# jason-gideon/GPUMounter

Hardware: AMD Instinct MI355X
Metric: p50_gpu_attach_latency_ms (lower is better)
Workload: dtype none

## Files before the change

### gpumounter_amd/_native.py

```python
from __future__ import annotations

import ctypes as C
import os
import subprocess
import threading
from typing import Optional

LIB_DIR = os.path.join(os.path.dirname(os.path.abspath(__file__)), "_lib")
NATIVE_DIR = os.path.join(os.path.dirname(os.path.dirname(os.path.abspath(__file__))), "native")

_lock = threading.Lock()
_libs: dict = {}


class NativeError(RuntimeError):
    pass


def lib_path(name: str) -> str:
    return os.path.join(LIB_DIR, name)


def build(target: str = "all", quiet: bool = True) -> None:
    import fcntl
# ... 79 lines not shown
    _fields_ = [("type", C.c_char), ("access", C.c_uint8), ("allow", C.c_uint8),
                ("pad", C.c_uint8), ("major", C.c_int32), ("minor", C.c_int32)]


class DevNode(C.Structure):
    _fields_ = [("path", C.c_char * 112), ("major", C.c_uint32), ("minor", C.c_uint32),
                ("mode", C.c_uint32), ("uid", C.c_int32), ("gid", C.c_int32)]


class BpfTiming(C.Structure):
    _fields_ = [("query_ns", C.c_uint64), ("map_ns", C.c_uint64), ("build_ns", C.c_uint64),
                ("load_ns", C.c_uint64), ("attach_ns", C.c_uint64), ("programs", C.c_uint32),
                ("insns", C.c_uint32)]


HOST_ABI_VERSION = 6
GM_ACC_MKNOD, GM_ACC_READ, GM_ACC_WRITE = 1, 2, 4
GM_DEV_EMULATE, GM_DEV_VIA_SETNS, GM_DEV_REPLACE, GM_DEV_BIND = 1, 2, 4, 8


def host() -> C.CDLL:
    lib = _load("libgm_host.so", "host")
    if not getattr(lib, "_gm_typed", False):
        abi = lib.gm_host_abi_version()
        if abi != HOST_ABI_VERSION:
            raise RuntimeError(f"libgm_host.so ABI {abi} != {HOST_ABI_VERSION} expected: stale "
                               f"build, run `make -C native`")
        lib.gm_cg1_apply.argtypes = [C.c_char_p, C.POINTER(DevRule), C.c_int]
        lib.gm_cg1_format_rule.argtypes = [C.POINTER(DevRule), C.c_char_p, C.c_int]
        lib.gm_bpf_dev_build.argtypes = [C.POINTER(DevRule), C.c_int, C.c_int, C.c_int,
                                         C.POINTER(C.c_uint64), C.c_int]
# ... 21 lines not shown
        lib.gm_bpf_dev_set_at.argtypes = [C.c_char_p, C.c_uint32, C.POINTER(C.c_uint32),
                                          C.c_uint32, C.POINTER(C.c_uint32),
                                          C.POINTER(C.c_uint32)]
        lib.gm_bpf_dev_last_timing.argtypes = [C.POINTER(BpfTiming)]
        lib.gm_bpf_dev_last_timing.restype = None
        lib.gm_devnodes_create.argtypes = [C.c_int, C.c_char_p, C.POINTER(DevNode), C.c_int,
                                           C.c_int, C.POINTER(C.c_int)]
        lib.gm_devnodes_remove.argtypes = lib.gm_devnodes_create.argtypes
        lib.gm_devnodes_guard.argtypes = [C.c_char_p]
        lib.gm_devnodes_stage.argtypes = [C.c_char_p, C.c_int]
        lib.gm_devnode_stat.argtypes = [C.c_int, C.c_char_p, C.c_char_p, C.c_int,
                                        C.POINTER(C.c_int), C.POINTER(C.c_uint32),
                                        C.POINTER(C.c_uint32), C.POINTER(C.c_uint32)]
        lib.gm_devnodes_present.argtypes = [C.c_int, C.c_char_p, C.POINTER(DevNode), C.c_int,
                                            C.c_int, C.POINTER(C.c_uint8)]
        lib.gm_proc_dev_users.argtypes = [C.c_uint32, C.c_uint32, C.POINTER(C.c_int32), C.c_int,
                                          C.POINTER(C.c_int)]
        lib.gm_proc_scan_devs.argtypes = [C.POINTER(C.c_int32), C.c_int, C.POINTER(C.c_uint32),
                                          C.c_int, C.POINTER(C.c_uint8), C.POINTER(C.c_int32)]
        lib.gm_proc_filter_dev_users.argtypes = [C.POINTER(C.c_int32), C.c_int, C.c_uint32,
                                                 C.c_uint32, C.POINTER(C.c_int32)]
        lib.gm_proc_read_pids.argtypes = [C.c_char_p, C.POINTER(C.c_int32), C.c_int,
                                          C.POINTER(C.c_int)]
        lib.gm_sd_get_device_allow.argtypes = [C.c_char_p, C.c_char_p, C.c_char_p, C.c_int,
                                               C.c_char_p, C.c_int]
        lib.gm_sd_set_device_allow.argtypes = [C.c_char_p, C.c_char_p, C.POINTER(C.c_char_p),
                                               C.POINTER(C.c_char_p), C.c_int, C.c_int,
                                               C.c_char_p, C.c_int]
        lib.gm_sd_unit_path.argtypes = [C.c_char_p, C.c_char_p, C.c_int]
        lib.gm_roctx_push.argtypes = [C.c_char_p]
# ... 217 lines not shown
```

### gpumounter_amd/node/cgroup.py

```python
from __future__ import annotations

import ctypes as C
import errno
import functools
import glob
import json
import os
from abc import ABC, abstractmethod
from typing import Dict, FrozenSet, Iterable, List, Optional, Sequence, Set, Tuple

from gpumounter_amd import _native
from gpumounter_amd.models.device import DeviceNode
from gpumounter_amd.models.pod import (QOS_BESTEFFORT, QOS_BURSTABLE, ContainerRef, qos_class,
                                       uid_of)
from gpumounter_amd.node import bpfvm
from gpumounter_amd.utils import log, trace

_log = log.get("node.cgroup")

RUNTIME_SCOPE_PREFIXES = ("cri-containerd-", "docker-", "crio-", "containerd-", "")
FAKE_MARKER = ".gm_fake"
BPF_STATE = "gm.bpf.json"


# ... 93 lines not shown
                ctrls = parts[1].split(",") if parts[1] else [""]
                if want_ctrl not in ctrls:
                    continue
                cand = os.path.join(self.base, parts[2].lstrip("/"))
                if os.path.isdir(cand):
                    return cand
        return None

    def forget(self, pod_uid: str) -> None:
        for k in [k for k in self._cache if k[0] == pod_uid]:
            del self._cache[k]

    @staticmethod
    def pids(cgdir: str, recursive: bool = True) -> List[int]:
        lib = _native.host()
        out: List[int] = []
        buf = (C.c_int32 * 4096)()
        n = C.c_int(0)
        stack = [cgdir]
        while stack:
            d = stack.pop()
            path = os.path.join(d, "cgroup.procs")
            rc = lib.gm_proc_read_pids(path.encode(), buf, 4096, C.byref(n))
            if rc < 0 and rc != -errno.ENOENT:
                raise CgroupError(f"read {path}: {os.strerror(-rc)}")
            if rc >= 0:
                out.extend(buf[:min(n.value, 4096)])
            if recursive:
                try:
                    with os.scandir(d) as it:
                        stack.extend(e.path for e in it if e.is_dir(follow_symlinks=False))
                except (FileNotFoundError, NotADirectoryError):
                    pass
        return sorted(set(out))


def rules_for(nodes: Iterable[DeviceNode], allow: bool, access: str = "rw") -> List[_native.DevRule]:
    acc = 0
    if "r" in access:
        acc |= _native.GM_ACC_READ
    if "w" in access:
        acc |= _native.GM_ACC_WRITE
    if "m" in access:
        acc |= _native.GM_ACC_MKNOD
    return [_native.DevRule(b"c", acc, 1 if allow else 0, 0, n.major, n.minor) for n in nodes]


def _rule_array(rules: Sequence[_native.DevRule]):
    arr = (_native.DevRule * max(len(rules), 1))()
# ... 442 lines not shown
```

### gpumounter_amd/node/devnodes.py

```python
from __future__ import annotations

import ctypes as C
import errno
import os
from dataclasses import dataclass
from typing import List, Optional, Sequence, Tuple

from gpumounter_amd import _native
from gpumounter_amd.models.device import DeviceNode
from gpumounter_amd.utils import log


class DevNodeError(RuntimeError):
    def __init__(self, msg: str, results: Sequence[int] = ()):
        super().__init__(msg)
        self.results = list(results)


@dataclass(frozen=True)
class Target:

    pid: int = 0
    root: str = ""


CREATED, PRESENT, SHARED_HOST = 0, 1, 2

_log = log.get("node.devnodes")


class DevNodeWriter:

    def __init__(self, mode: str = "procroot", host_dev: str = "", userns: str = "auto",
                 stage_dir: str = "", proc_root: str = "/proc") -> None:
        self.mode = mode
        self.userns = userns
        self.stage_dir = stage_dir
        self.proc_root = proc_root
        self._staged = False
        self._own_userns = self._userns_id("self")
        self.flags = 0
        if mode == "setns":
            self.flags |= _native.GM_DEV_VIA_SETNS
# ... 7 lines not shown

    @staticmethod
    def _array(nodes: Sequence[DeviceNode], owner: Tuple[int, int] = (-1, -1)):
        arr = (_native.DevNode * max(len(nodes), 1))()
        for i, n in enumerate(nodes):
            rel = n.path.lstrip("/").encode()
            if len(rel) >= 112:
                raise DevNodeError(f"path too long: {n.path}")
            arr[i].path = rel
            arr[i].major = n.major
            arr[i].minor = n.minor
            arr[i].mode = n.mode
            arr[i].uid, arr[i].gid = owner
        return arr

    def _mntns(self, pid) -> Optional[str]:
        try:
            return os.readlink(f"{self.proc_root}/{pid}/ns/mnt")
        except OSError:
            return None

    def root_pid(self, pids: Sequence[int]) -> int:
        if self.mode == "emulate":
            return pids[0] if pids else 0
        own = self._mntns("self")
        for pid in pids:
            ns = self._mntns(pid)
            if ns is not None and ns != own:
                return pid
        return 0

    def _userns_id(self, pid) -> Optional[Tuple[int, int]]:
        try:
            st = os.stat(f"{self.proc_root}/{pid}/ns/user")
        except OSError:
            return None
        return st.st_dev, st.st_ino

    def _bind(self, t: Target) -> bool:
        if self.userns == "bind":
            return True
        if self.userns != "auto" or self.mode == "emulate" or t.root or t.pid <= 0:
            return False
        theirs = self._userns_id(t.pid)
        return theirs is not None and self._own_userns is not None and theirs != self._own_userns
# ... 32 lines not shown
        self._staged = True

    def _call(self, t: Target):
        if not self._bind(t):
            return self.flags, (-1, -1)
        self._ensure_stage()
        return self.flags | _native.GM_DEV_BIND, self._mapped_root(t)

    def _target_args(self, t: Target) -> Tuple[int, Optional[bytes]]:
        if t.root:
            return 0, t.root.encode()
        if t.pid <= 0:
            raise DevNodeError("container has no process to resolve its root from "
                               "(empty cgroup.procs)")
        return t.pid, None

    def create(self, t: Target, nodes: Sequence[DeviceNode]) -> List[int]:
        if not nodes:
            return []
        pid, root = self._target_args(t)
        flags, owner = self._call(t)
        res = (C.c_int * len(nodes))()
        fails = _native.host().gm_devnodes_create(pid, root, self._array(nodes, owner),
                                                  len(nodes), flags, res)
        results = [int(res[i]) for i in range(len(nodes))]
        if fails:
            bad = [(n.path, os.strerror(-r)) for n, r in zip(nodes, results) if r < 0]
            what = "bind mount" if flags & _native.GM_DEV_BIND else "mknod"
            raise DevNodeError(f"{what} failed: {bad}", results)
        return results
# ... 44 lines not shown
        return kind in (1, 2) and ma == node.major and mi == node.minor

    def present_many(self, t: Target, nodes: Sequence[DeviceNode]) -> List[bool]:
        return [bool(s) for s in self.present_states(t, nodes)]

    def present_states(self, t: Target, nodes: Sequence[DeviceNode]) -> List[int]:
        if not nodes:
            return []
        pid, root = self._target_args(t)
        out = (C.c_uint8 * len(nodes))()
        rc = _native.host().gm_devnodes_present(pid, root, self._array(nodes), len(nodes),
                                                self._call(t)[0], out)
        if rc < 0:
            raise DevNodeError(f"read-back of {len(nodes)} nodes: {os.strerror(-rc)}")
        return [int(out[i]) for i in range(len(nodes))]
```

### gpumounter_amd/node/hotmount.py

```python
from __future__ import annotations

import os
from dataclasses import dataclass, field
from typing import Dict, List, Optional, Sequence

from gpumounter_amd.hw.inventory import Inventory
from gpumounter_amd.models.device import AmdGpu, DeviceNode, kfd_node
from gpumounter_amd.models.pod import ContainerRef, running_containers
from gpumounter_amd.node.cgroup import CgroupError, CgroupResolver, DeviceRuleBackend
from gpumounter_amd.node.devnodes import CREATED, DevNodeError, DevNodeWriter, Target
from gpumounter_amd.node.journal import InjectionJournal
from gpumounter_amd.utils import log, trace

_log = log.get("node.hotmount")


class MountError(RuntimeError):
    pass


@dataclass
class ContainerTarget:
    ref: ContainerRef
    cgdir: str
    target: Target
    pids: List[int] = field(default_factory=list)


@dataclass
class AuditIssue:
    container: str
    kind: str
    path: str
    major: int
    minor: int


class HotMount:
    def __init__(self, cfg, inv: Inventory, resolver: CgroupResolver, backend: DeviceRuleBackend,
                 writer: DevNodeWriter, faults=None,
                 journal: Optional[InjectionJournal] = None) -> None:
# ... 61 lines not shown
        try:
            return self.targets(pod, container, include_privileged)
        except (CgroupError, OSError) as e:
            raise MountError(f"cannot resolve the pod's containers: {e}") from e

    def attach(self, pod: dict, new: Sequence[AmdGpu], have: Sequence[AmdGpu],
               base: Sequence[AmdGpu] = (), container: str = "") -> List[ContainerTarget]:
        before = self.managed_nodes(have, base)
        after = self.managed_nodes(list(have) + list(new), base)
        before_keys = {(n.major, n.minor) for n in before}
        grant = [n for n in after if (n.major, n.minor) not in before_keys]
        with trace.span("resolve"):
            targets = self.resolve(pod, container)
        done: List[tuple] = []
        j = self.journal
        try:
            for t in targets:
                cid = t.ref.id
                known = j.nodes_of(cid)
                with trace.span("devnodes_probe", nodes=len(after)):
                    states = self.writer.present_states(t.target, after)
                theirs = {(n.major, n.minor) for n, st in zip(after, states)
                          if st and (n.major, n.minor) not in known}
                j.intend(cid, [((n.major, n.minor), n.path) for n in grant],
                         [((n.major, n.minor), n.path) for n in after
                          if (n.major, n.minor) not in theirs], **self._owner(pod, t))
                done.append((t, grant, []))
                with trace.span("cgroup_rule", backend=self.backend.name, rules=len(grant)):
                    self.faults.check("cgroup_rule")
                    self._apply(t.cgdir, grant, [], after)
                self.faults.check("cgroup_rule", "after")
                with trace.span("devnodes", nodes=len(after)):
                    self.faults.check("devnodes")
                    res = self.writer.create(t.target, after)
                done[-1] = (t, grant, [n for n, r in zip(after, res) if r == CREATED])
                j.settle(cid, [(n.major, n.minor) for n, r in zip(after, res)
                               if r != CREATED and (n.major, n.minor) not in known
                               and (n.major, n.minor) not in theirs])
                self.faults.check("devnodes", "after")
        except Exception as e:
            self._rollback_attach(done, before)
            for t in targets[len(done):]:
                self._forget_new(t.ref.id, grant, after, before)
            raise MountError(f"attach failed, rolled back: {e}") from e
        return targets

    def _forget_new(self, cid: str, granted, after, before) -> None:
        keep = {(n.major, n.minor) for n in before}
        self.journal.forget(cid, [(n.major, n.minor) for n in granted],
                            [(n.major, n.minor) for n in after if (n.major, n.minor) not in keep])

    def _rollback_attach(self, done, before: List[DeviceNode]) -> None:
        before_keys = {(n.major, n.minor) for n in before}
        for t, granted, created in reversed(done):
            try:
                self.writer.remove(t.target, created)
            except Exception as e:
                _log.error("rollback unlink in %s failed: %s", t.ref.name, e)
            else:
                self.journal.forget(t.ref.id, (), [(n.major, n.minor) for n in created
                                                   if (n.major, n.minor) not in before_keys])
# ... 108 lines not shown
        rules = [DeviceNode(p, ma, mi) for (ma, mi), p in sorted(ent.rules.items())]
        nodes = [DeviceNode(p, ma, mi) for (ma, mi), p in sorted(ent.nodes.items())]
        out = [AuditIssue(t.ref.name, "stale_rule", n.path, n.major, n.minor) for n in rules]
        out += [AuditIssue(t.ref.name, "stale_node", n.path, n.major, n.minor) for n in nodes]
        if rules:
            self._apply(t.cgdir, [], rules, [])
            self.journal.forget(container_id, [(n.major, n.minor) for n in rules])
        if nodes:
            self.writer.remove(t.target, nodes)
            self.journal.forget(container_id, (), [(n.major, n.minor) for n in nodes])
        return out

    def verify(self, pod: dict, hot: Sequence[AmdGpu], base: Sequence[AmdGpu] = (),
               container: str = "",
               targets: Optional[List[ContainerTarget]] = None) -> List[AuditIssue]:
        want = self.managed_nodes(hot, base)
        issues: List[AuditIssue] = []
        try:
            return self._verify(want, targets if targets is not None
                                else self.targets(pod, container), issues)
        except (CgroupError, DevNodeError, OSError) as e:
            raise MountError(f"read-back failed: {e}") from e

    def _verify(self, want: List[DeviceNode], targets: List[ContainerTarget],
                issues: List[AuditIssue]) -> List[AuditIssue]:
        for t in targets:
            allowed = self.backend.allowed(t.cgdir)
            present = self.writer.present_many(t.target, want)
            for n, ok in zip(want, present):
                if (n.major, n.minor) not in allowed:
                    issues.append(AuditIssue(t.ref.name, "missing_rule", n.path, n.major, n.minor))
                if not ok:
                    issues.append(AuditIssue(t.ref.name, "missing_node", n.path, n.major, n.minor))
        return issues

    def audit(self, pod: dict, hot: Sequence[AmdGpu], base: Sequence[AmdGpu] = (),
              container: str = "") -> List[AuditIssue]:
        want = self.managed_nodes(hot, base)
        want_keys = {(n.major, n.minor) for n in want}
        issues: List[AuditIssue] = []
        base_keys = {(n.major, n.minor) for n in self.gpu_nodes(base)}
        for t in self.targets(pod, container):
            allowed = self.backend.allowed(t.cgdir)
# ... 29 lines not shown
```

### gpumounter_amd/node/journal.py

```python
from __future__ import annotations

import json
import os
import threading
import time
from dataclasses import dataclass, field
from typing import Dict, Iterable, List, Optional, Tuple

from gpumounter_amd.utils import log

_log = log.get("node.journal")

Key = Tuple[int, int]


@dataclass
class Entry:
    container_id: str
    namespace: str = ""
    pod: str = ""
    pod_uid: str = ""
    container: str = ""
    cgdir: str = ""
    rules: Dict[Key, str] = field(default_factory=dict)
# ... 7 lines not shown
        return {"container_id": self.container_id, "namespace": self.namespace, "pod": self.pod,
                "pod_uid": self.pod_uid, "container": self.container, "cgdir": self.cgdir,
                "rules": sorted([ma, mi, p] for (ma, mi), p in self.rules.items()),
                "nodes": sorted([ma, mi, p] for (ma, mi), p in self.nodes.items()),
                "updated": self.updated}

    @classmethod
    def from_json(cls, d: dict) -> "Entry":
        return cls(d["container_id"], d.get("namespace", ""), d.get("pod", ""),
                   d.get("pod_uid", ""), d.get("container", ""), d.get("cgdir", ""),
                   {(int(a), int(b)): p for a, b, p in d.get("rules", [])},
                   {(int(a), int(b)): p for a, b, p in d.get("nodes", [])},
                   float(d.get("updated", 0.0)))


def _safe_id(cid: str) -> bool:
    return bool(cid) and all(c.isalnum() or c in "-_." for c in cid) and cid[0] != "."


class InjectionJournal:
    def __init__(self, state_dir: str = "") -> None:
        self.dir = state_dir
        self._entries: Dict[str, Entry] = {}
        self._mu = threading.Lock()
        self.writes = 0
        if state_dir:
            os.makedirs(state_dir, mode=0o700, exist_ok=True)
            self._load()

    def _path(self, cid: str) -> str:
        return os.path.join(self.dir, cid + ".json")

    def _load(self) -> None:
        for fn in os.listdir(self.dir):
            if not fn.endswith(".json"):
                continue
            try:
                with open(os.path.join(self.dir, fn), encoding="utf-8") as fh:
                    e = Entry.from_json(json.load(fh))
            except (OSError, ValueError, KeyError, TypeError) as ex:
                _log.error("journal: unreadable record %s (%s); ignoring it", fn, ex)
                continue
            if e.container_id + ".json" == fn:
                self._entries[e.container_id] = e

    def _store(self, e: Entry) -> None:
        self.writes += 1
        if not self.dir:
            return
        path = self._path(e.container_id)
        if e.empty():
            try:
                os.unlink(path)
            except FileNotFoundError:
                pass
            return
        tmp = path + ".tmp"
        blob = json.dumps(e.to_json(), separators=(",", ":")).encode()
        fd = os.open(tmp, os.O_WRONLY | os.O_CREAT | os.O_TRUNC | os.O_CLOEXEC, 0o600)
        try:
            view = memoryview(blob)
            while view:
                view = view[os.write(fd, view):]
        finally:
            os.close(fd)
        os.replace(tmp, path)

    def get(self, cid: str) -> Optional[Entry]:
        return self._entries.get(cid)

    def entries(self) -> List[Entry]:
        with self._mu:
            return list(self._entries.values())
# ... 20 lines not shown
                if v:
                    setattr(e, k, v)
        return e

    def intend(self, cid: str, rules: Iterable[Tuple[Key, str]] = (),
               nodes: Iterable[Tuple[Key, str]] = (), **owner: str) -> None:
        with self._mu:
            e = self._entry(cid, owner)
            before = (len(e.rules), len(e.nodes))
            e.rules.update(rules)
            e.nodes.update(nodes)
            if (len(e.rules), len(e.nodes)) != before or not e.updated:
                e.updated = time.time()
                self._store(e)

    def settle(self, cid: str, not_ours: Iterable[Key]) -> None:
        keys = list(not_ours)
        if not keys:
            return
        with self._mu:
            e = self._entries.get(cid)
            if e is None:
                return
            changed = False
            for k in keys:
                changed |= e.nodes.pop(k, None) is not None
            if changed:
                e.updated = time.time()
                self._store(e)

# ... 24 lines not shown
```

### native/include/gm_host.h

```cpp
#pragma once
#include <stdint.h>

#ifdef __cplusplus
extern "C" {
#endif

#define GM_HOST_ABI_VERSION 6

#define GM_ACC_MKNOD 1
#define GM_ACC_READ 2
#define GM_ACC_WRITE 4

typedef struct gm_dev_rule {
  char type;
  uint8_t access;
  uint8_t allow;
  uint8_t pad;
  int32_t major;
  int32_t minor;
} gm_dev_rule_t;

int gm_cg1_apply(const char* cgdir, const gm_dev_rule_t* rules, int n);
int gm_cg1_format_rule(const gm_dev_rule_t* rule, char* out, int cap);

// ... 38 lines not shown
#define GM_DEV_REPLACE 4
#define GM_DEV_BIND 8

int gm_devnodes_guard(const char* host_dev);
int gm_devnodes_stage(const char* dir, int mount_tmpfs);
int gm_devnodes_bind_probe(void);
int gm_devnodes_create(int pid, const char* root, const gm_dev_node_t* nodes, int n, int flags,
                       int* results);
int gm_devnodes_remove(int pid, const char* root, const gm_dev_node_t* nodes, int n, int flags,
                       int* results);
int gm_devnode_stat(int pid, const char* root, const char* path, int flags, int* kind,
                    uint32_t* major, uint32_t* minor, uint32_t* mode);
int gm_devnodes_present(int pid, const char* root, const gm_dev_node_t* nodes, int n, int flags,
                        uint8_t* present);

int gm_proc_dev_users(uint32_t major, uint32_t minor, int32_t* pids, int cap, int* n);
int gm_proc_scan_devs(const int32_t* pids, int n, const uint32_t* majmin, int ndev,
                      uint8_t* hits, int32_t* unreadable);
int gm_proc_filter_dev_users(const int32_t* pids, int n, uint32_t major, uint32_t minor,
                             int32_t* out);
int gm_proc_read_pids(const char* path, int32_t* pids, int cap, int* n);

int gm_sd_get_device_allow(const char* bus_path, const char* unit, char* out, int cap, char* err,
                           int errcap);
int gm_sd_set_device_allow(const char* bus_path, const char* unit, const char* const* paths,
                           const char* const* perms, int n, int reset, char* err, int errcap);
int gm_sd_unit_path(const char* unit, char* out, int cap);

int gm_roctx_available(void);
void gm_roctx_push(const char* name);
void gm_roctx_pop(void);
void gm_roctx_mark(const char* name);
uint64_t gm_roctx_start(const char* name);
void gm_roctx_stop(uint64_t id);
uint64_t gm_now_ns(void);

// ... 6 lines not shown
```

### native/src/gm_host.cpp

```cpp
#include "gm_host.h"

#include <dirent.h>
#include <dlfcn.h>
#include <errno.h>
#include <fcntl.h>
#include <linux/bpf.h>
#include <sched.h>
#include <signal.h>
#include <stdio.h>
#include <stdlib.h>
#include <string.h>
#include <sys/mount.h>
#include <sys/stat.h>
#include <sys/syscall.h>
#include <sys/sysmacros.h>
#include <time.h>
#include <unistd.h>

#include <atomic>
#include <map>
#include <mutex>
#include <string>
#include <thread>
#include <vector>

namespace {

constexpr const char* kProgName = "gm_devallow";

struct Fd {
  int fd = -1;
  Fd() = default;
  explicit Fd(int f) : fd(f) {}
// ... 814 lines not shown
  if (kind == 0) return 1;
  int mounted = is_mount_leaf(pfd, leaf);
  if (mounted < 0) return mounted;
  if (!mounted) {
    if (kind == 3 && is_placeholder(pfd, leaf)) {
      if (unlinkat(pfd, leaf.c_str(), 0) < 0) return -errno;
      return 0;
    }
    return remove_one(w, n);
  }
  if (!(kind == 1 && maj == n.major && min == n.minor)) return -EEXIST;
  if ((e = unmount_leaf(pfd, leaf)) < 0) return e;
  if (is_placeholder(pfd, leaf) && unlinkat(pfd, leaf.c_str(), 0) < 0) return -errno;
  return 0;
}

struct Roctx {
  std::once_flag once;
  int (*push)(const char*) = nullptr;
  int (*pop)() = nullptr;
  void (*mark)(const char*) = nullptr;
  uint64_t (*start)(const char*) = nullptr;
  void (*stop)(uint64_t) = nullptr;
};
Roctx g_roctx;

void roctx_init() {
  std::call_once(g_roctx.once, []() {
    const char* env = getenv("GM_ROCTX");
    if (env && strcmp(env, "0") == 0) return;
// ... 230 lines not shown
  memset(&a, 0, sizeof(a));
  a.info.bpf_fd = (uint32_t)pfd.fd;
  a.info.info_len = sizeof(info);
  a.info.info = ptr_u64(&info);
  if (sys_bpf(BPF_OBJ_GET_INFO_BY_FD, &a, sizeof(a)) < 0) return -errno;
  return 0;
}

int gm_bpf_dev_program(const char* cgroup_path, uint64_t* insns, uint32_t cap, uint32_t* n,
                       uint32_t* prog_id) {
  return gm_bpf_dev_program_at(cgroup_path, 0, 0, insns, cap, n, prog_id, nullptr);
}

namespace {
thread_local gm_bpf_timing_t t_bpf_timing;
uint64_t mono_ns() {
  struct timespec ts;
  clock_gettime(CLOCK_MONOTONIC, &ts);
  return (uint64_t)ts.tv_sec * 1000000000ull + (uint64_t)ts.tv_nsec;
}
}

void gm_bpf_dev_last_timing(gm_bpf_timing_t* out) {
  if (out) *out = t_bpf_timing;
}

int gm_bpf_dev_install(const char* cgroup_path, const gm_dev_rule_t* rules, int n,
                       const gm_dev_rule_t* base, int nbase, const char* pin_dir,
                       uint32_t* prog_id, uint32_t* chained_id) {
  gm_bpf_timing_t& tm = t_bpf_timing;
  tm = gm_bpf_timing_t{};
  uint64_t t0 = mono_ns();
  Fd cg(open(cgroup_path, O_RDONLY | O_DIRECTORY | O_CLOEXEC));
  if (!cg.ok()) return -errno;
  const uint64_t ino = cgroup_ino(cg.fd);
// ... 300 lines not shown
    if (e == -ENOENT) {
      *kind = 0;
      *maj = *min = *mode = 0;
      return 0;
    }
    if (e < 0) return e;
    return stat_leaf(parent.fd, leaf, kind, maj, min, mode);
  });
}

int gm_devnodes_present(int pid, const char* root, const gm_dev_node_t* nodes, int n, int flags,
                        uint8_t* present) {
  int count = 0;
  int e = with_root(pid, root, flags, [&](int rootfd) {
    Walker wk(rootfd);
    for (int i = 0; i < n; ++i) {
      present[i] = 0;
      int pfd;
      std::string leaf;
      int w = wk.parent(nodes[i].path, false, &pfd, &leaf);
      if (w == -ENOENT) {
        std::string dir(nodes[i].path);
        const size_t cut = dir.rfind('/');
        dir = cut == std::string::npos ? std::string() : dir.substr(0, cut);
        Fd d2;
        std::string l2;
        if (!dir.empty() && walk_parent(rootfd, dir.c_str(), false, &d2, &l2) == 0 &&
            guarded_dir(d2.fd)) {
          present[i] = kSharedHost;
          ++count;
        }
        continue;
      }
      if (w < 0) continue;
      if (guarded_dir(pfd)) {
        present[i] = kSharedHost;
        ++count;
        continue;
      }
      int kind = 0;
      uint32_t ma = 0, mi = 0, mode = 0;
      if (stat_leaf(pfd, leaf, &kind, &ma, &mi, &mode) < 0) continue;
      if ((kind == 1 || kind == 2) && ma == nodes[i].major && mi == nodes[i].minor &&
          (!(flags & GM_DEV_BIND) || is_mount_leaf(pfd, leaf) == 1)) {
        present[i] = 1;
        ++count;
      }
    }
    return 0;
  });
  return e < 0 ? e : count;
}

namespace {
bool pid_uses_dev(long pid, dev_t want) {
  char p[64];
  snprintf(p, sizeof(p), "/proc/%ld/fd", pid);
  int dfd = open(p, O_RDONLY | O_DIRECTORY | O_CLOEXEC);
  if (dfd < 0) return false;
  DIR* fds = fdopendir(dfd);
  if (!fds) {
    close(dfd);
    return false;
  }
  struct dirent* fe;
  bool hit = false;
  while (!hit && (fe = readdir(fds)) != nullptr) {
// ... 70 lines not shown
}

int gm_proc_read_pids(const char* path, int32_t* pids, int cap, int* n) {
  *n = 0;
  FILE* f = fopen(path, "re");
  if (!f) return -errno;
  long v;
  while (fscanf(f, "%ld", &v) == 1) {
    if (*n < cap) pids[*n] = (int32_t)v;
    ++*n;
  }
  fclose(f);
  return 0;
}

int gm_roctx_available(void) {
  roctx_init();
  return g_roctx.push != nullptr;
}
void gm_roctx_push(const char* name) {
  roctx_init();
  if (g_roctx.push) g_roctx.push(name);
}
void gm_roctx_pop(void) {
  roctx_init();
  if (g_roctx.pop) g_roctx.pop();
}
uint64_t gm_roctx_start(const char* name) {
  roctx_init();
  return g_roctx.start ? g_roctx.start(name) : 0;
// ... 17 lines not shown
```

Baseline: 1.098.

## Add native stepped attach path fusing probe, journal write, mknod and readback

Adds a native attach handle that opens the container root once, probes node presence, optionally writes the journal record, then creates nodes and reads back presence in a single context. The Python attach loop uses it when the writer is plain, and verify reuses the carried presence instead of re-probing. The cgroup pid walk and root-pid mount-namespace resolution also move into C. The aim is to cut repeated root opens, path walks and Python/ctypes overhead per attach, at the cost of a larger native surface, an ABI bump and staleness risk when carried state is reused.

```diff
diff --git a/gpumounter_amd/_native.py b/gpumounter_amd/_native.py
--- a/gpumounter_amd/_native.py
+++ b/gpumounter_amd/_native.py
@@ -117,7 +117,7 @@
                 ("insns", C.c_uint32)]
 
 
-HOST_ABI_VERSION = 6
+HOST_ABI_VERSION = 7
 GM_ACC_MKNOD, GM_ACC_READ, GM_ACC_WRITE = 1, 2, 4
 GM_DEV_EMULATE, GM_DEV_VIA_SETNS, GM_DEV_REPLACE, GM_DEV_BIND = 1, 2, 4, 8
 
@@ -169,6 +169,19 @@
                                         C.POINTER(C.c_uint32), C.POINTER(C.c_uint32)]
         lib.gm_devnodes_present.argtypes = [C.c_int, C.c_char_p, C.POINTER(DevNode), C.c_int,
                                             C.c_int, C.POINTER(C.c_uint8)]
+        lib.gm_attach_begin.argtypes = [C.c_int, C.c_char_p, C.POINTER(DevNode), C.c_int,
+                                        C.c_int, C.POINTER(C.c_uint8), C.POINTER(C.c_void_p)]
+        lib.gm_attach_begin_journal.argtypes = [C.c_int, C.c_char_p, C.POINTER(DevNode), C.c_int,
+                                                C.c_int, C.POINTER(C.c_uint8), C.c_char_p,
+                                                C.c_char_p, C.c_uint32, C.POINTER(C.c_uint8),
+                                                C.POINTER(C.c_int), C.POINTER(C.c_void_p)]
+        lib.gm_attach_journal.argtypes = [C.c_void_p, C.c_char_p, C.c_char_p, C.c_uint32]
+        lib.gm_attach_finish.argtypes = [C.c_void_p, C.POINTER(C.c_int), C.POINTER(C.c_uint8),
+                                         C.POINTER(C.c_uint64)]
+        lib.gm_attach_close.argtypes = [C.c_void_p]
+        lib.gm_attach_close.restype = None
+        lib.gm_cg_procs.argtypes = [C.c_char_p, C.c_char_p, C.c_int, C.POINTER(C.c_int32),
+                                    C.c_int, C.POINTER(C.c_int), C.POINTER(C.c_int32)]
         lib.gm_proc_dev_users.argtypes = [C.c_uint32, C.c_uint32, C.POINTER(C.c_int32), C.c_int,
                                           C.POINTER(C.c_int)]
         lib.gm_proc_scan_devs.argtypes = [C.POINTER(C.c_int32), C.c_int, C.POINTER(C.c_uint32),
diff --git a/gpumounter_amd/node/cgroup.py b/gpumounter_amd/node/cgroup.py
--- a/gpumounter_amd/node/cgroup.py
+++ b/gpumounter_amd/node/cgroup.py
@@ -131,25 +131,24 @@
     @staticmethod
     def pids(cgdir: str, recursive: bool = True) -> List[int]:
         lib = _native.host()
-        out: List[int] = []
+        n = C.c_int(0)
+        if recursive:
+            cap = 4096
+            while True:
+                buf = (C.c_int32 * cap)()
+                rc = lib.gm_cg_procs(cgdir.encode(), None, 0, buf, cap, C.byref(n), None)
+                if rc != -errno.ENOSPC:
+                    break
+                cap = n.value
+            if rc < 0:
+                raise CgroupError(f"read cgroup.procs below {cgdir}: {os.strerror(-rc)}")
+            return buf[:n.value]
         buf = (C.c_int32 * 4096)()
-        n = C.c_int(0)
-        stack = [cgdir]
-        while stack:
-            d = stack.pop()
-            path = os.path.join(d, "cgroup.procs")
-            rc = lib.gm_proc_read_pids(path.encode(), buf, 4096, C.byref(n))
-            if rc < 0 and rc != -errno.ENOENT:
-                raise CgroupError(f"read {path}: {os.strerror(-rc)}")
-            if rc >= 0:
-                out.extend(buf[:min(n.value, 4096)])
-            if recursive:
-                try:
-                    with os.scandir(d) as it:
-                        stack.extend(e.path for e in it if e.is_dir(follow_symlinks=False))
-                except (FileNotFoundError, NotADirectoryError):
-                    pass
-        return sorted(set(out))
+        path = os.path.join(cgdir, "cgroup.procs")
+        rc = lib.gm_proc_read_pids(path.encode(), buf, 4096, C.byref(n))
+        if rc < 0 and rc != -errno.ENOENT:
+            raise CgroupError(f"read {path}: {os.strerror(-rc)}")
+        return sorted(set(buf[:min(n.value, 4096)])) if rc >= 0 else []
 
 
 def rules_for(nodes: Iterable[DeviceNode], allow: bool, access: str = "rw") -> List[_native.DevRule]:
diff --git a/gpumounter_amd/node/devnodes.py b/gpumounter_amd/node/devnodes.py
--- a/gpumounter_amd/node/devnodes.py
+++ b/gpumounter_amd/node/devnodes.py
@@ -27,6 +27,36 @@
 CREATED, PRESENT, SHARED_HOST = 0, 1, 2
 
 _log = log.get("node.devnodes")
+
+
+class AttachStep:
+
+    __slots__ = ("_lib", "_h", "n", "states", "journaled")
+
+    def __init__(self, lib, handle, n: int, states: List[int], journaled: bool) -> None:
+        self._lib, self._h, self.n, self.states, self.journaled = lib, handle, n, states, journaled
+
+    def journal(self, path: str, blob: bytes) -> None:
+        rc = self._lib.gm_attach_journal(self._h, path.encode(), blob, len(blob))
+        if rc < 0:
+            raise OSError(-rc, os.strerror(-rc), path)
+
+    def finish(self, nodes: Sequence[DeviceNode]) -> Tuple[List[int], List[int]]:
+        res = (C.c_int * self.n)()
+        after = (C.c_uint8 * self.n)()
+        fails = self._lib.gm_attach_finish(self._h, res, after, None)
+        results = list(res)
+        if fails:
+            if fails < 0:
+                results = [fails] * self.n
+            bad = [(n.path, os.strerror(-r)) for n, r in zip(nodes, results) if r < 0]
+            raise DevNodeError(f"mknod failed: {bad}", results)
+        return results, list(after)
+
+    def close(self) -> None:
+        h, self._h = self._h, None
+        if h:
+            self._lib.gm_attach_close(h)
 
 
 class DevNodeWriter:
@@ -64,21 +94,18 @@
             arr[i].uid, arr[i].gid = owner
         return arr
 
-    def _mntns(self, pid) -> Optional[str]:
-        try:
-            return os.readlink(f"{self.proc_root}/{pid}/ns/mnt")
-        except OSError:
-            return None
-
     def root_pid(self, pids: Sequence[int]) -> int:
         if self.mode == "emulate":
             return pids[0] if pids else 0
-        own = self._mntns("self")
-        for pid in pids:
-            ns = self._mntns(pid)
-            if ns is not None and ns != own:
-                return pid
-        return 0
+        if not pids:
+            return 0
+        n, root = C.c_int(len(pids)), C.c_int32(0)
+        rc = _native.host().gm_cg_procs(None, self.proc_root.encode(), 1,
+                                        (C.c_int32 * len(pids))(*pids), len(pids),
+                                        C.byref(n), C.byref(root))
+        if rc < 0:
+            raise DevNodeError(f"resolving the container's root process: {os.strerror(-rc)}")
+        return root.value
 
     def _userns_id(self, pid) -> Optional[Tuple[int, int]]:
         try:
@@ -141,6 +168,32 @@
             raise DevNodeError("container has no process to resolve its root from "
                                "(empty cgroup.procs)")
         return t.pid, None
+
+    def steppable(self, t: Target) -> bool:
+        if self.flags & _native.GM_DEV_VIA_SETNS and not t.root:
+            return False
+        return not self._bind(t)
+
+    def begin(self, t: Target, nodes: Sequence[DeviceNode], known: Sequence[bool] = (),
+              path: Optional[str] = None, blob: Optional[bytes] = None) -> Optional[AttachStep]:
+        pid, root = self._target_args(t)
+        n = len(nodes)
+        states = (C.c_uint8 * n)()
+        mask = (C.c_uint8 * n)(*known) if known else None
+        journaled = C.c_int(0)
+        handle = C.c_void_p()
+        lib = _native.host()
+        rc = lib.gm_attach_begin_journal(pid, root, self._array(nodes), n, self.flags, mask,
+                                         path.encode() if path else None, blob,
+                                         len(blob) if blob else 0, states, C.byref(journaled),
+                                         C.byref(handle))
+        if rc == -errno.ENOTSUP:
+            return None
+        if rc < 0:
+            if journaled.value < 0:
+                raise OSError(-rc, os.strerror(-rc), path)
+            raise DevNodeError(f"read-back of {n} nodes: {os.strerror(-rc)}")
+        return AttachStep(lib, handle, n, list(states), journaled.value == 1)
 
     def create(self, t: Target, nodes: Sequence[DeviceNode]) -> List[int]:
         if not nodes:
@@ -215,3 +268,15 @@
         if rc < 0:
             raise DevNodeError(f"read-back of {len(nodes)} nodes: {os.strerror(-rc)}")
         return [int(out[i]) for i in range(len(nodes))]
+
+
+_STEPPED = ("present_states", "present_many", "create")
+_STEPPED_IMPL = tuple(DevNodeWriter.__dict__[m] for m in _STEPPED)
+
+
+def plain_writer(w) -> bool:
+    if type(w) is not DevNodeWriter:
+        return False
+    own = w.__dict__
+    return not any(m in own for m in _STEPPED) and \
+        all(DevNodeWriter.__dict__.get(m) is f for m, f in zip(_STEPPED, _STEPPED_IMPL))
diff --git a/gpumounter_amd/node/hotmount.py b/gpumounter_amd/node/hotmount.py
--- a/gpumounter_amd/node/hotmount.py
+++ b/gpumounter_amd/node/hotmount.py
@@ -8,11 +8,14 @@
 from gpumounter_amd.models.device import AmdGpu, DeviceNode, kfd_node
 from gpumounter_amd.models.pod import ContainerRef, running_containers
 from gpumounter_amd.node.cgroup import CgroupError, CgroupResolver, DeviceRuleBackend
-from gpumounter_amd.node.devnodes import CREATED, DevNodeError, DevNodeWriter, Target
+from gpumounter_amd.node.devnodes import (CREATED, DevNodeError, DevNodeWriter, Target,
+                                          plain_writer)
 from gpumounter_amd.node.journal import InjectionJournal
 from gpumounter_amd.utils import log, trace
 
 _log = log.get("node.hotmount")
+
+FAST_ATTACH = True
 
 
 class MountError(RuntimeError):
@@ -25,6 +28,7 @@
     cgdir: str
     target: Target
     pids: List[int] = field(default_factory=list)
+    carry: Optional[tuple] = field(default=None, compare=False, repr=False)
 
 
 @dataclass
@@ -116,8 +120,11 @@
             targets = self.resolve(pod, container)
         done: List[tuple] = []
         j = self.journal
+        carry_key = ([g.index for g in have] + [g.index for g in new], [g.index for g in base])
         try:
             for t in targets:
+                if self._fast(t) and self._attach_fast(pod, t, grant, after, done, carry_key):
+                    continue
                 cid = t.ref.id
                 known = j.nodes_of(cid)
                 with trace.span("devnodes_probe", nodes=len(after)):
@@ -147,6 +154,46 @@
             raise MountError(f"attach failed, rolled back: {e}") from e
         return targets
 
+    def _fast(self, t: ContainerTarget) -> bool:
+        return FAST_ATTACH and plain_writer(self.writer) and not self.faults \
+            and self.writer.steppable(t.target)
+
+    def _attach_fast(self, pod: dict, t: ContainerTarget, grant: List[DeviceNode],
+                     after: List[DeviceNode], done: List[tuple], carry_key: tuple) -> bool:
+        if not after:
+            return False
+        j = self.journal
+        cid = t.ref.id
+        known = j.nodes_of(cid)
+        keys = [(n.major, n.minor) for n in after]
+        rules = [((n.major, n.minor), n.path) for n in grant]
+        owner = self._owner(pod, t)
+        plan = j.plan(cid, rules, [(k, n.path) for k, n in zip(keys, after)], **owner)
+        with trace.span("devnodes_probe", nodes=len(after)):
+            step = self.writer.begin(t.target, after, [k in known for k in keys],
+                                     plan.path, plan.blob)
+        if step is None:
+            return False
+        try:
+            theirs = {k for k, st in zip(keys, step.states) if st and k not in known}
+            if not theirs:
+                j.commit(plan, stored=step.journaled)
+            else:
+                j.commit(j.plan(cid, rules, [(k, n.path) for k, n in zip(keys, after)
+                                             if k not in theirs], **owner), writer=step.journal)
+            done.append((t, grant, []))
+            with trace.span("cgroup_rule", backend=self.backend.name, rules=len(grant)):
+                self._apply(t.cgdir, grant, [], after)
+            with trace.span("devnodes", nodes=len(after)):
+                res, present = step.finish(after)
+            done[-1] = (t, grant, [n for n, r in zip(after, res) if r == CREATED])
+            j.settle(cid, [k for k, r in zip(keys, res)
+                           if r != CREATED and k not in known and k not in theirs])
+            t.carry = (carry_key[0], carry_key[1], after, present)
+        finally:
+            step.close()
+        return True
+
     def _forget_new(self, cid: str, granted, after, before) -> None:
         keep = {(n.major, n.minor) for n in before}
         self.journal.forget(cid, [(n.major, n.minor) for n in granted],
@@ -285,19 +332,30 @@
     def verify(self, pod: dict, hot: Sequence[AmdGpu], base: Sequence[AmdGpu] = (),
                container: str = "",
                targets: Optional[List[ContainerTarget]] = None) -> List[AuditIssue]:
-        want = self.managed_nodes(hot, base)
+        key = ([g.index for g in hot], [g.index for g in base])
+        carried = [getattr(t, "carry", None) for t in targets or ()]
+        if carried and all(c is not None and (c[0], c[1]) == key for c in carried):
+            want = carried[0][2]
+        else:
+            want = self.managed_nodes(hot, base)
         issues: List[AuditIssue] = []
         try:
             return self._verify(want, targets if targets is not None
-                                else self.targets(pod, container), issues)
+                                else self.targets(pod, container), issues, key)
         except (CgroupError, DevNodeError, OSError) as e:
             raise MountError(f"read-back failed: {e}") from e
 
     def _verify(self, want: List[DeviceNode], targets: List[ContainerTarget],
-                issues: List[AuditIssue]) -> List[AuditIssue]:
+                issues: List[AuditIssue], key: Optional[tuple] = None) -> List[AuditIssue]:
         for t in targets:
             allowed = self.backend.allowed(t.cgdir)
-            present = self.writer.present_many(t.target, want)
+            carry = getattr(t, "carry", None)
+            if carry is not None:
+                t.carry = None
+            if carry is not None and (carry[0], carry[1]) == key and len(carry[3]) == len(want):
+                present = [bool(s) for s in carry[3]]
+            else:
+                present = self.writer.present_many(t.target, want)
             for n, ok in zip(want, present):
                 if (n.major, n.minor) not in allowed:
                     issues.append(AuditIssue(t.ref.name, "missing_rule", n.path, n.major, n.minor))
diff --git a/gpumounter_amd/node/journal.py b/gpumounter_amd/node/journal.py
--- a/gpumounter_amd/node/journal.py
+++ b/gpumounter_amd/node/journal.py
@@ -2,6 +2,7 @@
 
 import json
 import os
+import re
 import threading
 import time
 from dataclasses import dataclass, field
@@ -45,8 +46,23 @@
                    float(d.get("updated", 0.0)))
 
 
+_SAFE_ID = re.compile(r"(?!\.)[\w.\-]+")
+
+
 def _safe_id(cid: str) -> bool:
-    return bool(cid) and all(c.isalnum() or c in "-_." for c in cid) and cid[0] != "."
+    return _SAFE_ID.fullmatch(cid) is not None
+
+
+@dataclass
+class Intent:
+    cid: str
+    rules: List[Tuple[Key, str]]
+    nodes: List[Tuple[Key, str]]
+    owner: Dict[str, str]
+    basis: tuple
+    updated: float = 0.0
+    path: Optional[str] = None
+    blob: Optional[bytes] = None
 
 
 class InjectionJournal:
@@ -75,7 +91,12 @@
             if e.container_id + ".json" == fn:
                 self._entries[e.container_id] = e
 
-    def _store(self, e: Entry) -> None:
+    @staticmethod
+    def _blob(e: Entry) -> bytes:
+        return json.dumps(e.to_json(), separators=(",", ":")).encode()
+
+    def _store(self, e: Entry, blob: Optional[bytes] = None, stored: bool = False,
+               writer=None) -> None:
         self.writes += 1
         if not self.dir:
             return
@@ -86,8 +107,14 @@
             except FileNotFoundError:
                 pass
             return
+        if stored:
+            return
+        if blob is None:
+            blob = self._blob(e)
+        if writer is not None:
+            writer(path, blob)
+            return
         tmp = path + ".tmp"
-        blob = json.dumps(e.to_json(), separators=(",", ":")).encode()
         fd = os.open(tmp, os.O_WRONLY | os.O_CREAT | os.O_TRUNC | os.O_CLOEXEC, 0o600)
         try:
             view = memoryview(blob)
@@ -138,6 +165,46 @@
                 e.updated = time.time()
                 self._store(e)
 
+    @staticmethod
+    def _basis(e: Optional[Entry]) -> tuple:
+        return (e, 0, 0, 0.0) if e is None else (e, len(e.rules), len(e.nodes), e.updated)
+
+    def plan(self, cid: str, rules: Iterable[Tuple[Key, str]] = (),
+             nodes: Iterable[Tuple[Key, str]] = (), **owner: str) -> Intent:
+        if not _safe_id(cid):
+            raise ValueError(f"journal: bad container id {cid!r}")
+        with self._mu:
+            e = self._entries.get(cid)
+            it = Intent(cid, list(rules), list(nodes), owner, self._basis(e))
+            new = Entry(cid) if e is None else Entry(cid, e.namespace, e.pod, e.pod_uid,
+                                                     e.container, e.cgdir, dict(e.rules),
+                                                     dict(e.nodes), e.updated)
+            for k, v in owner.items():
+                if v:
+                    setattr(new, k, v)
+            new.rules.update(it.rules)
+            new.nodes.update(it.nodes)
+            if (len(new.rules), len(new.nodes)) != it.basis[1:3] or not new.updated:
+                it.updated = new.updated = time.time()
+                if self.dir and not new.empty():
+                    it.path, it.blob = self._path(cid), self._blob(new)
+            return it
+
+    def commit(self, it: Intent, stored: bool = False, writer=None) -> None:
+        with self._mu:
+            fresh = self._basis(self._entries.get(it.cid)) == it.basis
+            e = self._entry(it.cid, it.owner)
+            before = (len(e.rules), len(e.nodes))
+            e.rules.update(it.rules)
+            e.nodes.update(it.nodes)
+            if (len(e.rules), len(e.nodes)) != before or not e.updated:
+                if fresh and it.updated:
+                    e.updated = it.updated
+                    self._store(e, it.blob, stored and it.blob is not None, writer)
+                else:
+                    e.updated = time.time()
+                    self._store(e, writer=writer)
+
     def settle(self, cid: str, not_ours: Iterable[Key]) -> None:
         keys = list(not_ours)
         if not keys:
diff --git a/native/include/gm_host.h b/native/include/gm_host.h
--- a/native/include/gm_host.h
+++ b/native/include/gm_host.h
@@ -5,7 +5,7 @@
 extern "C" {
 #endif
 
-#define GM_HOST_ABI_VERSION 6
+#define GM_HOST_ABI_VERSION 7
 
 #define GM_ACC_MKNOD 1
 #define GM_ACC_READ 2
@@ -76,12 +76,24 @@
 int gm_devnodes_present(int pid, const char* root, const gm_dev_node_t* nodes, int n, int flags,
                         uint8_t* present);
 
+typedef struct gm_attach gm_attach_t;
+int gm_attach_begin(int pid, const char* root, const gm_dev_node_t* nodes, int n, int flags,
+                    uint8_t* states, gm_attach_t** out);
+int gm_attach_begin_journal(int pid, const char* root, const gm_dev_node_t* nodes, int n,
+                            int flags, const uint8_t* known, const char* path, const void* blob,
+                            uint32_t len, uint8_t* states, int* journaled, gm_attach_t** out);
+int gm_attach_journal(gm_attach_t* ctx, const char* path, const void* blob, uint32_t len);
+int gm_attach_finish(gm_attach_t* ctx, int* results, uint8_t* present_after, uint64_t ns[2]);
+void gm_attach_close(gm_attach_t* ctx);
+
 int gm_proc_dev_users(uint32_t major, uint32_t minor, int32_t* pids, int cap, int* n);
 int gm_proc_scan_devs(const int32_t* pids, int n, const uint32_t* majmin, int ndev,
                       uint8_t* hits, int32_t* unreadable);
 int gm_proc_filter_dev_users(const int32_t* pids, int n, uint32_t major, uint32_t minor,
                              int32_t* out);
 int gm_proc_read_pids(const char* path, int32_t* pids, int cap, int* n);
+int gm_cg_procs(const char* cgdir, const char* proc_root, int pick_root, int32_t* pids, int cap,
+                int* n, int32_t* root_pid);
 
 int gm_sd_get_device_allow(const char* bus_path, const char* unit, char* out, int cap, char* err,
                            int errcap);
diff --git a/native/src/gm_host.cpp b/native/src/gm_host.cpp
--- a/native/src/gm_host.cpp
+++ b/native/src/gm_host.cpp
@@ -17,6 +17,7 @@
 #include <time.h>
 #include <unistd.h>
 
+#include <algorithm>
 #include <atomic>
 #include <map>
 #include <mutex>
@@ -861,6 +862,76 @@
   if (is_placeholder(pfd, leaf) && unlinkat(pfd, leaf.c_str(), 0) < 0) return -errno;
   return 0;
 }
+
+int present_all(Walker& wk, const gm_dev_node_t* nodes, int n, int flags, uint8_t* present) {
+  int count = 0;
+  for (int i = 0; i < n; ++i) {
+    present[i] = 0;
+    int pfd;
+    std::string leaf;
+    int w = wk.parent(nodes[i].path, false, &pfd, &leaf);
+    if (w == -ENOENT) {
+      std::string dir(nodes[i].path);
+      const size_t cut = dir.rfind('/');
+      dir = cut == std::string::npos ? std::string() : dir.substr(0, cut);
+      Fd d2;
+      std::string l2;
+      if (!dir.empty() && walk_parent(wk.rootfd, dir.c_str(), false, &d2, &l2) == 0 &&
+          guarded_dir(d2.fd)) {
+        present[i] = kSharedHost;
+        ++count;
+      }
+      continue;
+    }
+    if (w < 0) continue;
+    if (guarded_dir(pfd)) {
+      present[i] = kSharedHost;
+      ++count;
+      continue;
+    }
+    int kind = 0;
+    uint32_t ma = 0, mi = 0, mode = 0;
+    if (stat_leaf(pfd, leaf, &kind, &ma, &mi, &mode) < 0) continue;
+    if ((kind == 1 || kind == 2) && ma == nodes[i].major && mi == nodes[i].minor &&
+        (!(flags & GM_DEV_BIND) || is_mount_leaf(pfd, leaf) == 1)) {
+      present[i] = 1;
+      ++count;
+    }
+  }
+  return count;
+}
+
+int store_record(const char* path, const void* blob, uint32_t len) {
+  if (!path || !*path || (!blob && len)) return -EINVAL;
+  const std::string tmp = std::string(path) + ".tmp";
+  int fd = open(tmp.c_str(), O_WRONLY | O_CREAT | O_TRUNC | O_CLOEXEC, 0600);
+  if (fd < 0) return -errno;
+  int e = write_all(fd, static_cast<const char*>(blob), len);
+  close(fd);
+  if (e < 0) return e;
+  return rename(tmp.c_str(), path) < 0 ? -errno : 0;
+}
+
+uint64_t mono_ns() {
+  struct timespec ts;
+  clock_gettime(CLOCK_MONOTONIC, &ts);
+  return (uint64_t)ts.tv_sec * 1000000000ull + (uint64_t)ts.tv_nsec;
+}
+
+}
+
+struct gm_attach {
+  Fd root;
+  Walker walker;
+  std::string root_path;
+  dev_t root_dev = 0;
+  ino_t root_ino = 0;
+  int flags = 0;
+  std::vector<gm_dev_node_t> nodes;
+  gm_attach(int rootfd, int fl) : root(rootfd), walker(rootfd), flags(fl) {}
+};
+
+namespace {
 
 struct Roctx {
   std::once_flag once;
@@ -1121,11 +1192,6 @@
 
 namespace {
 thread_local gm_bpf_timing_t t_bpf_timing;
-uint64_t mono_ns() {
-  struct timespec ts;
-  clock_gettime(CLOCK_MONOTONIC, &ts);
-  return (uint64_t)ts.tv_sec * 1000000000ull + (uint64_t)ts.tv_nsec;
-}
 }
 
 void gm_bpf_dev_last_timing(gm_bpf_timing_t* out) {
@@ -1456,43 +1522,100 @@
   int count = 0;
   int e = with_root(pid, root, flags, [&](int rootfd) {
     Walker wk(rootfd);
-    for (int i = 0; i < n; ++i) {
-      present[i] = 0;
-      int pfd;
-      std::string leaf;
-      int w = wk.parent(nodes[i].path, false, &pfd, &leaf);
-      if (w == -ENOENT) {
-        std::string dir(nodes[i].path);
-        const size_t cut = dir.rfind('/');
-        dir = cut == std::string::npos ? std::string() : dir.substr(0, cut);
-        Fd d2;
-        std::string l2;
-        if (!dir.empty() && walk_parent(rootfd, dir.c_str(), false, &d2, &l2) == 0 &&
-            guarded_dir(d2.fd)) {
-          present[i] = kSharedHost;
-          ++count;
-        }
-        continue;
-      }
-      if (w < 0) continue;
-      if (guarded_dir(pfd)) {
-        present[i] = kSharedHost;
-        ++count;
-        continue;
-      }
-      int kind = 0;
-      uint32_t ma = 0, mi = 0, mode = 0;
-      if (stat_leaf(pfd, leaf, &kind, &ma, &mi, &mode) < 0) continue;
-      if ((kind == 1 || kind == 2) && ma == nodes[i].major && mi == nodes[i].minor &&
-          (!(flags & GM_DEV_BIND) || is_mount_leaf(pfd, leaf) == 1)) {
-        present[i] = 1;
-        ++count;
-      }
-    }
+    count = present_all(wk, nodes, n, flags, present);
     return 0;
   });
   return e < 0 ? e : count;
 }
+
+int gm_attach_begin_journal(int pid, const char* root, const gm_dev_node_t* nodes, int n,
+                            int flags, const uint8_t* known, const char* path, const void* blob,
+                            uint32_t len, uint8_t* states, int* journaled, gm_attach_t** out) {
+  if (!out) return -EINVAL;
+  *out = nullptr;
+  if (journaled) *journaled = 0;
+  if (n < 0 || (n > 0 && (!nodes || !states))) return -EINVAL;
+  const bool explicit_root = root && *root;
+  if ((flags & GM_DEV_BIND) || ((flags & GM_DEV_VIA_SETNS) && !explicit_root)) return -ENOTSUP;
+  int rfd = open_root(pid, root);
+  if (rfd < 0) return rfd;
+  gm_attach* c = new gm_attach(rfd, flags);
+  struct stat st;
+  if (fstat(rfd, &st) < 0) {
+    int e = -errno;
+    delete c;
+    return e;
+  }
+  c->root_dev = st.st_dev;
+  c->root_ino = st.st_ino;
+  if (explicit_root) {
+    c->root_path = root;
+  } else {
+    char p[64];
+    snprintf(p, sizeof(p), "/proc/%d/root", pid);
+    c->root_path = p;
+  }
+  c->nodes.assign(nodes, nodes + n);
+  for (auto& nd : c->nodes) nd.path[sizeof(nd.path) - 1] = 0;
+  present_all(c->walker, c->nodes.data(), n, flags, states);
+  if (path && *path) {
+    bool foreign = false;
+    for (int i = 0; i < n && !foreign; ++i) foreign = states[i] && !(known && known[i]);
+    if (!foreign) {
+      int e = store_record(path, blob, len);
+      if (journaled) *journaled = e < 0 ? e : 1;
+      if (e < 0) {
+        delete c;
+        return e;
+      }
+    }
+  }
+  *out = c;
+  return 0;
+}
+
+int gm_attach_begin(int pid, const char* root, const gm_dev_node_t* nodes, int n, int flags,
+                    uint8_t* states, gm_attach_t** out) {
+  return gm_attach_begin_journal(pid, root, nodes, n, flags, nullptr, nullptr, nullptr, 0, states,
+                                 nullptr, out);
+}
+
+int gm_attach_journal(gm_attach_t* ctx, const char* path, const void* blob, uint32_t len) {
+  if (!ctx) return -EINVAL;
+  return store_record(path, blob, len);
+}
+
+int gm_attach_finish(gm_attach_t* ctx, int* results, uint8_t* present_after, uint64_t ns[2]) {
+  if (!ctx || !results || !present_after) return -EINVAL;
+  const int n = (int)ctx->nodes.size();
+  if (ns) ns[0] = ns[1] = 0;
+  const uint64_t t0 = mono_ns();
+  struct stat st;
+  int e = 0;
+  if (stat(ctx->root_path.c_str(), &st) < 0) e = -errno;
+  else if (st.st_dev != ctx->root_dev || st.st_ino != ctx->root_ino) e = -ESRCH;
+  if (e < 0) {
+    for (int i = 0; i < n; ++i) {
+      results[i] = e;
+      present_after[i] = 0;
+    }
+    return n;
+  }
+  int failures = 0;
+  for (int i = 0; i < n; ++i) {
+    results[i] = create_one(ctx->walker, ctx->nodes[i], ctx->flags);
+    if (results[i] < 0) ++failures;
+  }
+  const uint64_t t1 = mono_ns();
+  present_all(ctx->walker, ctx->nodes.data(), n, ctx->flags, present_after);
+  if (ns) {
+    ns[0] = t1 - t0;
+    ns[1] = mono_ns() - t1;
+  }
+  return failures;
+}
+
+void gm_attach_close(gm_attach_t* ctx) { delete ctx; }
 
 namespace {
 bool pid_uses_dev(long pid, dev_t want) {
@@ -1593,6 +1716,75 @@
   return 0;
 }
 
+namespace {
+int cg_walk(const std::string& dir, std::vector<int32_t>* out) {
+  const std::string procs = dir + "/cgroup.procs";
+  if (FILE* f = fopen(procs.c_str(), "re")) {
+    long v;
+    while (fscanf(f, "%ld", &v) == 1) out->push_back((int32_t)v);
+    fclose(f);
+  } else if (errno != ENOENT) {
+    return -errno;
+  }
+  DIR* d = opendir(dir.c_str());
+  if (!d) return errno == ENOENT || errno == ENOTDIR ? 0 : -errno;
+  std::vector<std::string> subs;
+  while (struct dirent* de = readdir(d)) {
+    const char* nm = de->d_name;
+    if (nm[0] == '.' && (nm[1] == 0 || (nm[1] == '.' && nm[2] == 0))) continue;
+    bool is_dir = de->d_type == DT_DIR;
+    if (de->d_type == DT_UNKNOWN) {
+      struct stat st;
+      is_dir = fstatat(dirfd(d), nm, &st, AT_SYMLINK_NOFOLLOW) == 0 && S_ISDIR(st.st_mode);
+    }
+    if (is_dir) subs.push_back(dir + "/" + nm);
+  }
+  closedir(d);
+  for (const std::string& s : subs) {
+    int e = cg_walk(s, out);
+    if (e < 0) return e;
+  }
+  return 0;
+}
+
+std::string link_of(const std::string& path) {
+  char buf[128];
+  ssize_t r = readlink(path.c_str(), buf, sizeof(buf) - 1);
+  return r < 0 ? std::string() : std::string(buf, (size_t)r);
+}
+}
+
+int gm_cg_procs(const char* cgdir, const char* proc_root, int pick_root, int32_t* pids, int cap,
+                int* n, int32_t* root_pid) {
+  if (!n || cap < 0 || (cap > 0 && !pids)) return -EINVAL;
+  if (root_pid) *root_pid = 0;
+  std::vector<int32_t> all;
+  if (cgdir) {
+    int e = cg_walk(cgdir, &all);
+    if (e < 0) return e;
+    std::sort(all.begin(), all.end());
+    all.erase(std::unique(all.begin(), all.end()), all.end());
+    *n = (int)all.size();
+    if ((int)all.size() > cap) return -ENOSPC;
+    if (!all.empty()) memcpy(pids, all.data(), all.size() * sizeof(int32_t));
+  } else {
+    if (*n < 0 || *n > cap) return -EINVAL;
+    all.assign(pids, pids + *n);
+  }
+  if (pick_root && root_pid) {
+    const std::string base = proc_root && *proc_root ? proc_root : "/proc";
+    const std::string own = link_of(base + "/self/ns/mnt");
+    for (int32_t pid : all) {
+      const std::string ns = link_of(base + "/" + std::to_string(pid) + "/ns/mnt");
+      if (!ns.empty() && ns != own) {
+        *root_pid = pid;
+        break;
+      }
+    }
+  }
+  return 0;
+}
+
 int gm_roctx_available(void) {
   roctx_init();
   return g_roctx.push != nullptr;
```

Result: slower. 1.184 (+7.8%).
